# drowe67/pirip

Measured on AMD Instinct MI355X. Metric: IQ Msamples/s demodulated (2-FSK Fs=240k Rs=10k); BER vs CPU ref, higher is better.
Workload: dtype f32

## Files before the change

### pirip_amd/csrc/fsk_demod_wave.hip

```cpp
#include <hip/hip_runtime.h>

#include <cmath>
#include <cstdio>
#include <cstdlib>

#include "../../include/pirip_hip.h"
#include "demod_simd.hpp"
#include "fsk_device.hpp"

namespace pirip {

namespace {

constexpr int kWave = 64;

struct cf { float x, y; };

__device__ __forceinline__ float add_lane_up(float a, float b)
{
    float r;
    asm("v_add_f32_dpp %0, %1, %2 wave_shl:1 row_mask:0xf bank_mask:0xf bound_ctrl:0" : "=v"(r) : "v"(a), "v"(b));
    return r;
}

// ... 62 lines not shown
{
    const float hi = x * 0.00133514404296875f;
    return __builtin_fmaf(x, -0x1.e60f04p-20f, hi);
}
template <int FMT>
__device__ __forceinline__ v2f decode(const uint32_t *rw, int k)
{
    if (FMT == PIRIP_IN_CU8_FSKDEMOD || FMT == PIRIP_IN_CU8_CSDR) {
        const uint32_t v = rw[k >> 1];
        return cvt_u8_pair<FMT>(v2f{(k & 1) ? ubyte2(v) : ubyte0(v), (k & 1) ? ubyte3(v) : ubyte1(v)});
    } else if (FMT == PIRIP_IN_CS16) {
        const uint32_t v = rw[k];
        return v2f{cvt_s16((float)(short)(v & 0xffffu)), cvt_s16((float)((int)v >> 16))};
    } else {
        return v2f{__builtin_bit_cast(float, rw[2 * k]), __builtin_bit_cast(float, rw[2 * k + 1])};
    }
}
template <int FMT>
__device__ __forceinline__ v2f lds_sample(const unsigned char *p)
{
    if (FMT == PIRIP_IN_CU8_FSKDEMOD || FMT == PIRIP_IN_CU8_CSDR) {
        const uint32_t v = *(const uint16_t *)p;
        return cvt_u8_pair<FMT>(v2f{ubyte0(v), ubyte1(v)});
    } else if (FMT == PIRIP_IN_CS16) {
        const uint32_t v = *(const uint32_t *)p;
        return v2f{cvt_s16((float)(short)(v & 0xffffu)), cvt_s16((float)((int)v >> 16))};
    } else {
        const float2 v = *(const float2 *)p;
        return v2f{v.x, v.y};
    }
}

constexpr int cmax(int a, int b) { return a > b ? a : b; }

__device__ __forceinline__ float atan2_turns(float y, float x)
{
    const float ax = fabsf(x), ay = fabsf(y);
    const float mn = ax < ay ? ax : ay, mx = ax < ay ? ay : ax;
    const float t = mx > 0.f ? mn * __builtin_amdgcn_rcpf(mx) : 0.f;
    const float s1 = t * t, s2 = s1 * s1, s4 = s2 * s2;
    const float p01 = __builtin_fmaf(s1, -0.05304612219333649f, 0.15915483236312866f);
    const float p23 = __builtin_fmaf(s1, -0.02213626727461815f, 0.031745944172143936f);
    const float p45 = __builtin_fmaf(s1, -0.00889870710670948f, 0.015346021391451359f);
    const float p67 = __builtin_fmaf(s1, -0.0006453014793805778f, 0.0034795869141817093f);
    const float q0 = __builtin_fmaf(s2, p23, p01), q1 = __builtin_fmaf(s2, p67, p45);
    float r = __builtin_fmaf(s4, q1, q0) * t;
    r = ay > ax ? 0.25f - r : r;
    r = x < 0.f ? 0.5f - r : r;
    return __builtin_copysignf(r, y);
}

constexpr float kLlrMax = 24.0f;
__device__ __forceinline__ float ln_i0_tab(const float *tab, float x)
{
    const bool in = x < 32.0f;
    const float xs = (in ? x : 32.0f) * 8.0f;
    const int j = (int)xs;
    const float f = xs - (float)j;
    const float t0 = tab[j], t1 = tab[j + 1];
    return (t0 + (f * (t1 - t0))) + (in ? 0.0f : x - 32.0f);
}
__device__ __forceinline__ uint32_t spread16(uint32_t x)
{
    x = (x | (x << 8)) & 0x00FF00FFu; x = (x | (x << 4)) & 0x0F0F0F0Fu; x = (x | (x << 2)) & 0x33333333u; x = (x | (x << 1)) & 0x55555555u;
    return x;
}
// ... 33 lines not shown
    static constexpr int TAIL_DW = HIST * BPS / 4;
    static constexpr int TRAILER_DW = GUARD_B / 4;
    static_assert((HIST * BPS) % 4 == 0 && (GUARD_B - HIST * BPS) % 4 == 0, "tail copies move whole dwords");
    static_assert(GUARD_B + (2 * M + 1) * 4 <= M * HIST * 8, "the state block holds the raw tail and its trailer");
    static constexpr int CHS = (BPS == 2) ? TS : (TS % 8 == 0 ? 8 : TS % 4 == 0 ? 4 : 2);
    static constexpr int CH_DW = CHS * BPS / 4;
    static_assert(TS % 2 == 0 && TS % P == 0 && P >= 4, "bad Ts / P");
    static_assert(NLANES <= kWave, "one lane per symbol block");
    static_assert((TS * BPS) % 16 == 0 && (CHS * BPS) % 16 == 0 && TS % CHS == 0, "block and chunk strides keep 16-byte alignment");
    static_assert((N + Q) / (NDFT / 2) - 1 == NFFT && N / (NDFT / 2) - 1 == NFFT, "numffts must not depend on nin");
    static_assert(NDFT == 256 ? (NFFT >= 4) : NDFT == 512 ? (NFFT % 2 == 0) : (NDFT == 128 && NFFT <= 8),
                  "FFT batches (Ndft = 256: the last batch of 4 may be partial; Ndft = 128: one batch of up to eight)");
    static_assert((NFFT - 1) * (NDFT / 2) + NDFT <= N - Q, "FFT windows stay inside the shortest frame");
    static_assert(M * P <= 48, "window prefix sums are kept in registers");
};

template <class C, int M> constexpr int wave_lds_bytes() { return C::RAW_B + C::XP_B; }

}

template <int M, int TS, int P, int NSYM, int NDFT, int FMT, int WPB, int WPS, bool FFT_FMA = false, bool MASK = false, int BAND = 0>
__global__ __launch_bounds__(kWave * WPB, WPS) void fsk_demod_wave_kernel(DemodArgs a_kernarg, int nstreams)
{
    constexpr bool INPLACE = TS == 10;
    static_assert(offsetof(DemodArgs, d) == 0, "the argument block is the first kernel argument");
    auto ap = [&]() {
        if constexpr (INPLACE) return (const __attribute__((address_space(4))) DemodArgs *)__builtin_amdgcn_kernarg_segment_ptr();
        else return (const DemodArgs *)&a_kernarg;
    }();
#define PIRIP_ARGS_REREAD() do { if constexpr (INPLACE) asm volatile("" : "+s"(ap)); } while (0)
#define a (*ap)
#define d (ap->d)
    static_assert(BAND == 0 || ((BAND == 2 || BAND == 4) && NDFT == 256 && !MASK), "band-only estimator: Ndft = 256, peak method, 32 or 64 bins");
    auto cmul = [](v2f x, v2f t) { return FFT_FMA ? rot_step(x, t) : cmul_x(x, t); };
    using C = WaveCfg<M, TS, P, NSYM, NDFT, FMT>;
    constexpr int N = C::N, NMEM = C::NMEM, HIST = C::HIST, STEP = C::STEP, Q = C::Q, BPS = C::BPS;
    constexpr int GUARD_B = C::GUARD_B;

    __shared__ __attribute__((aligned(16))) unsigned char s_raw[WPB][C::RAW_B];
    __shared__ __attribute__((aligned(16))) unsigned char s_xp[WPB][C::XP_B];
    constexpr int TAB_F = NDFT == 256 ? 12 * 16 * 4 : NDFT == 512 ? 8 * 16 * 2 + 12 * 32 * 2 : 8 * 16 * 2;
    __shared__ __attribute__((aligned(16))) float s_tab[TAB_F];
    __shared__ __attribute__((aligned(16))) float2 s_tph[P];
    __shared__ __attribute__((aligned(16))) float2 s_tgain[NSYM + 2];
    __shared__ float s_misc[WPB][3];
    extern __shared__ __attribute__((aligned(16))) float s_lnI0[];

    const int lane0 = threadIdx.x & (kWave - 1);
    const int wv = __builtin_amdgcn_readfirstlane(threadIdx.x >> 6);
    const int sid = blockIdx.x * WPB + wv;

    if (NDFT == 256) {
        for (int i = threadIdx.x; i < 12 * 16; i += kWave * WPB)
            ((float4 *)s_tab)[i] = ((const float4 *)a.t.fast_tab)[(i & 15) * 12 + (i >> 4)];
    } else {
        for (int i = threadIdx.x; i < TAB_F / 4; i += kWave * WPB) ((float4 *)s_tab)[i] = ((const float4 *)(a.t.fast_tab + NDFT))[i];
    }
    if constexpr (P <= 10) if (a.io.soft.llr) {
        if (a.io.soft.llr_map == kLlrRician) { for (int i = threadIdx.x; i < 258; i += kWave * WPB) s_lnI0[i] = a.io.soft.lnI0[i]; }
        else if (threadIdx.x < 20) {
            const int sg = threadIdx.x >> 2, cc = threadIdx.x & 3;
            const float c2 = sg == 0 ? 0.226f : sg == 1 ? 0.1245f : sg == 2 ? 0.0288f : sg == 3 ? 0.002f : 0.0f;
            const float c1 = sg == 0 ? 0.0125f : sg == 1 ? 0.2177f : sg == 2 ? 0.6314f : sg == 3 ? 0.9048f : 0.9867f;
            const float c0 = sg == 0 ? -0.0012f : sg == 1 ? -0.108f : sg == 2 ? -0.5645f : sg == 3 ? -1.2997f : -2.2053f;
            s_lnI0[threadIdx.x] = cc == 0 ? c2 : cc == 1 ? c1 : cc == 2 ? c0 : 0.0f;
        }
// ... 550 lines not shown
            }
#pragma unroll
            for (int x = 1; x < M; x++)
#pragma unroll
                for (int y = x; y > 0; y--)
                    if (freqi[y] < freqi[y - 1]) { const int t = freqi[y]; freqi[y] = freqi[y - 1]; freqi[y - 1] = t; }
        }
        constexpr int LOG2N = NDFT == 128 ? 7 : NDFT == 256 ? 8 : 9;
        uint32_t dthv[M];
        int tix[M];
#pragma unroll
        for (int m = 0; m < M; m++) {
            if constexpr (MASK) { dthv[m] = a.t.mask_dtheta[bb * M + m]; tix[m] = bb * M + m; }
            else { dthv[m] = (uint32_t)freqi[m] << (32 - LOG2N); tix[m] = freqi[m] + NDFT / 2; }
        }

        auto phasor = [&](uint32_t th) {
            const float2 w = a.t.tw[th >> (32 - LOG2N)];
            float pc = w.x, ps = -w.y;
            if constexpr (MASK) {
                const float bl = (float)(th & ((1u << (32 - LOG2N)) - 1u)) * 1.4629180792671596e-9f;
                const float b2 = bl * bl;
                const float cb = 1.0f - b2 * (0.5f - b2 * (1.0f / 24.0f));
                const float sb = bl * (1.0f - b2 * ((1.0f / 6.0f) - b2 * (1.0f / 120.0f)));
                const float c2 = pc * cb - ps * sb, s2 = ps * cb + pc * sb;
                pc = c2; ps = s2;
            }
            return make_float2(pc, ps);
        };
        __builtin_amdgcn_sched_barrier(0);
        PIRIP_T_MARK(2);
        v2f fi[M][P];
        v2f tot[M];
        {
            PIRIP_PHASE_LANE(lane);
            const int lb = lane < C::NLANES ? lane : C::NLANES - 1;
            const int boff = GUARD_B + (TS * lb - nold) * BPS;
            const int al = (GUARD_B - nold * BPS) & 15;
            v2f ph[M], dph[M], acc[M];
            v2f sw_ph[M], sw_dph[M];
            const int n0 = TS * lb - nold + 1;
            const int nold_blk = nold - TS * lb;
            const bool oldl = nold_blk > 0;
#pragma unroll
            for (int m = 0; m < M; m++) {
                const float2 stn = a.t.osc_step[tix[m]], stp = a.t.osc_step[tixp[m]];
                const float dn = a.t.osc_drift[tix[m]].x, dp = a.t.osc_drift[tixp[m]].x;
                const uint32_t th = (uint32_t)n0 * (oldl ? dthp[m] : dthv[m]);
                const float g = 1.0f + (oldl ? dp * (float)(ninp + n0) : dn * (float)n0);
                const float2 pcs = phasor(th);
                ph[m] = v2f{pcs.x * g, pcs.y * g};
                dph[m] = oldl ? v2f{stp.x, stp.y} : v2f{stn.x, stn.y};
                const float2 p1 = phasor(dthv[m]);
                const float g1 = 1.0f + dn;
                sw_ph[m] = v2f{p1.x * g1, p1.y * g1};
                sw_dph[m] = v2f{stn.x, stn.y};
                acc[m] = v2f{0.f, 0.f};
            }
            const int zero_blk = ninp ? 0 : nold_blk;
#pragma unroll
            for (int c = 0; c < TS / C::CHS; c++) {
                uint32_t rw[C::CH_DW];
                if (C::DIRECT && lb >= 3) {
#pragma unroll
                    for (int i = 0; i < C::CH_DW / 4; i++) {
                        const auto v = __builtin_amdgcn_raw_buffer_load_b128(rsrc, (TS * lb - nold) * BPS + c * C::CHS * BPS + 16 * i, (int)goff_frame, 0);
                        const uint4 u = __builtin_bit_cast(uint4, v);
// ... 49 lines not shown
                    if ((kk & 3) == 3) __builtin_amdgcn_sched_barrier(0);
                }
            }
#pragma unroll
            for (int m = 0; m < M; m++) tot[m] = acc[m];
        }
        PIRIP_PHASE_LANE(lane);
        if constexpr (C::DIRECT) {
            asm volatile("s_waitcnt lgkmcnt(0)" ::: "memory");
            wave_lds_sync();
            const uint32_t toff = (uint32_t)__builtin_amdgcn_readfirstlane((int)(uint32_t)((pos + nin - HIST) * BPS));
#pragma unroll
            for (int i = 0; i < (C::TAIL_DW + kWave - 1) / kWave; i++)
                if (lane + i * kWave < C::TAIL_DW)
                    __builtin_amdgcn_raw_ptr_buffer_load_lds(rsrc, (lds_ptr)(raw + GUARD_B - HIST * BPS + i * 256), 4, lane * 4, toff + i * 256, 0, 0);
        } else {
            const uint32_t *tsrc = (const uint32_t *)(raw + GUARD_B + (nin - HIST) * BPS);
            uint32_t *tdst = (uint32_t *)(raw + GUARD_B - HIST * BPS);
            uint32_t tv[(C::TAIL_DW + kWave - 1) / kWave];
#pragma unroll
            for (int i = 0; i < (C::TAIL_DW + kWave - 1) / kWave; i++) tv[i] = tsrc[lane + i * kWave < C::TAIL_DW ? lane + i * kWave : 0];
#pragma unroll
            for (int i = 0; i < (C::TAIL_DW + kWave - 1) / kWave; i++) if (lane + i * kWave < C::TAIL_DW) tdst[lane + i * kWave] = tv[i];
        }
        asm volatile("s_waitcnt lgkmcnt(0)" ::: "memory");
        wave_lds_sync();
        PIRIP_T_MARK(3);
        dma_frame(pos + nin);
        ninp = nin;
#pragma unroll
        for (int m = 0; m < M; m++) { dthp[m] = dthv[m]; tixp[m] = tix[m]; }

        float tcr = 0.f, tci = 0.f;
        {
            v2f prpi{0.f, 0.f};
            v2f ft{0.f, 0.f};
#pragma unroll
            for (int q = 0; q < P; q++) {
#pragma unroll
                for (int m = 0; m < M; m++) {
                    const v2f own = fi[m][q];
                    v2f w0;
                    w0.x = add_lane_up(own.x, tot[m].x - own.x);
                    w0.y = add_lane_up(own.y, tot[m].y - own.y);
                    fi[m][q] = w0;
                    if (m == 0) asm("v_mul_f32 %0, %1, %1\n\tv_fma_f32 %0, %2, %2, %0" : "=&v"(ft.x) : "v"(w0.y), "v"(w0.x));
                    else { float t2; asm("v_mul_f32 %0, %2, %2\n\tv_fma_f32 %0, %3, %3, %0\n\tv_add_f32 %1, %1, %0" : "=&v"(t2), "+v"(ft.x) : "v"(w0.y), "v"(w0.x)); }
                }
                const v2f tp = *(const v2f *)&s_tph[q];
                asm("v_pk_fma_f32 %0, %1, %2, %0 op_sel_hi:[0,1,1]" : "+v"(prpi) : "v"(ft), "v"(tp));
                asm volatile("" : "+v"(prpi), "+v"(fi[0][q]), "+v"(fi[M - 1][q]));
            }
            const float pr = prpi.x, pi = prpi.y;
            if (lane <= NSYM) {
                const float2 tgain = s_tgain[lane];
                tcr = pr * tgain.x - pi * tgain.y;
                tci = pr * tgain.y + pi * tgain.x;
            }
            tcr = wave_sum(tcr); tci = wave_sum(tci);
        }

        PIRIP_T_MARK(4);
        PIRIP_ARGS_REREAD();
        const int frame_bytes = d.pack_bits ? (d.Nbits + 7) / 8 : d.Nbits;
        const size_t orow = (size_t)(frame + out0);
        uint8_t *bits_o = a.io.bits ? a.io.bits + (size_t)sid * a.io.bits_stride + orow * frame_bytes : nullptr;
        float *filt_o = a.io.filt ? a.io.filt + (size_t)sid * a.io.filt_stride + orow * M * NSYM : nullptr;
        float *stats_o = a.io.stats ? a.io.stats + (size_t)sid * a.io.stats_stride + orow * PIRIP_STATS_PER_FRAME : nullptr;
        float f_est[kMaxTones] = {0.f, 0.f, 0.f, 0.f};
#pragma unroll
        for (int m = 0; m < M; m++) {
            if constexpr (MASK) f_est[m] = (float)((bb - NDFT / 2) * d.Fs / NDFT) + (float)(m * d.tone_spacing);
            else f_est[m] = (float)freqi[m] * d.bin_hz;
        }

        const bool bad = isnan(tcr) || isnan(tci);
        int nin_next = nin;
        if (!bad) {
            const float norm_rx_timing = FMT == PIRIP_IN_CF32 ? atan2f(tci, tcr) * 0.15915494309189535f : atan2_turns(tci, tcr);
            const float rx_timing = norm_rx_timing * (float)P;
            const float d_norm = norm_rx_timing - sc_norm_rx_timing;
            sc_norm_rx_timing = norm_rx_timing;
            if (fabsf(d_norm) < 0.2f) {
                const float appm = (1e6f * d_norm) / (float)NSYM;
                sc_ppm = (0.9f * sc_ppm) + (0.1f * appm);
            }
            nin_next = N;
            if (!d.burst_mode) {
                if (norm_rx_timing > 0.25f) nin_next = N + Q;
                else if (norm_rx_timing < -0.25f) nin_next = N - Q;
            }

            const int low_sample = __builtin_amdgcn_readfirstlane((int)floorf(rx_timing));
            const float fract = rx_timing - (float)low_sample;
            const int high_sample = __builtin_amdgcn_readfirstlane((int)ceilf(rx_timing));
            v2f lo[M], hi[M];
            {
                const int ql = low_sample >= 0 ? low_sample : P + low_sample;
                const int qh = high_sample >= 0 ? high_sample : P + high_sample;
#define PIRIP_SEL_CASE(q) case q: if (q < P) { asm volatile(""); for (int m_ = 0; m_ < M; m_++) DST[m_] = fi[m_][q < P ? q : 0]; } break;
#define PIRIP_SELECT(idx) do { switch (idx) { \
    PIRIP_SEL_CASE(0) PIRIP_SEL_CASE(1) PIRIP_SEL_CASE(2) PIRIP_SEL_CASE(3) PIRIP_SEL_CASE(4) PIRIP_SEL_CASE(5) \
    PIRIP_SEL_CASE(6) PIRIP_SEL_CASE(7) PIRIP_SEL_CASE(8) PIRIP_SEL_CASE(9) PIRIP_SEL_CASE(10) PIRIP_SEL_CASE(11) \
    PIRIP_SEL_CASE(12) PIRIP_SEL_CASE(13) PIRIP_SEL_CASE(14) PIRIP_SEL_CASE(15) PIRIP_SEL_CASE(16) PIRIP_SEL_CASE(17) \
    PIRIP_SEL_CASE(18) PIRIP_SEL_CASE(19) PIRIP_SEL_CASE(20) PIRIP_SEL_CASE(21) PIRIP_SEL_CASE(22) PIRIP_SEL_CASE(23) \
    default: break; } } while (0)
                static_assert(P <= 24, "selection switch covers 24 window starts");
#pragma unroll
                for (int m = 0; m < M; m++) { lo[m] = fi[m][0]; hi[m] = fi[m][0]; }
#define DST lo
                PIRIP_SELECT(ql);
#undef DST
#define DST hi
                PIRIP_SELECT(qh);
#undef DST
#undef PIRIP_SELECT
#undef PIRIP_SEL_CASE
#pragma unroll
                for (int m = 0; m < M; m++) {
                    if (low_sample >= 0) { lo[m].x = lane_up(lo[m].x); lo[m].y = lane_up(lo[m].y); }
                    if (high_sample >= 0) { hi[m].x = lane_up(hi[m].x); hi[m].y = lane_up(hi[m].y); }
                }
            }
            float tmax[M];
            float sum = 0.f;
#pragma unroll
            for (int m = 0; m < M; m++) {
                v2f t;
                t.x = (1 - fract) * lo[m].x; t.y = (1 - fract) * lo[m].y;
                t.x = t.x + fract * hi[m].x; t.y = t.y + fract * hi[m].y;
// ... 132 lines not shown
        frame++;
        wave_lds_sync();
    }

    if constexpr (SOFT_OK) if (words_o && soft_cb > 0 && lane0 == 0) words_o[soft_w] = soft_carry;
    asm volatile("s_waitcnt vmcnt(0)" ::: "memory");
#ifdef PIRIP_WAVE_TIMING
    if (a.io.stats && lane0 == 0 && sid == nstreams / 2)
        for (int i = 0; i < 8; i++) a.io.stats[(size_t)sid * a.io.stats_stride + i] = (float)t_acc_[i];
#endif
#pragma unroll
    for (int b = 0; b < NB; b++) if (!BAND || lane0 < 16) a.s.Sf[(size_t)sid * NDFT + own_sfi(lane0, b)] = Sf[b];
    wave_lds_sync();
    for (int i = lane0; i < GUARD_B / 4; i += kWave) st32[i] = ((const uint32_t *)raw)[i];
    const int lane = lane0;
    if (lane == 0) {
#pragma unroll
        for (int m = 0; m < M; m++) { st32[C::TRAILER_DW + m] = dthp[m]; st32[C::TRAILER_DW + M + m] = (uint32_t)tixp[m]; }
        st32[C::TRAILER_DW + 2 * M] = (uint32_t)ninp;
        StreamScalars sc = a.s.scal[sid];
        sc.nin = nin; sc.norm_rx_timing = sc_norm_rx_timing; sc.ppm = sc_ppm; sc.SNRest = sc_SNRest;
        sc.snr_est = s_misc[wv][0]; sc.EbNodB = s_misc[wv][1]; sc.v_est = s_misc[wv][2];
        if (frame > frame_first) {
            const int fq[4] = {last_freqi0, last_freqi1, last_freqi2, last_freqi3};
            for (int m = 0; m < kMaxTones; m++) {
                if (MASK) sc.f_est[m] = m < M ? (float)((fq[0] - NDFT / 2) * d.Fs / NDFT) + (float)(m * d.tone_spacing) : 0.f;
                else sc.f_est[m] = m < M ? (float)fq[m] * d.bin_hz : 0.f;
            }
        }
        a.s.scal[sid] = sc;
        if (a.io.nframes) a.io.nframes[sid] = (int32_t)frame;
        if (a.io.consumed) a.io.consumed[sid] = pos;
    }
#undef a
#undef d
#undef PIRIP_ARGS_REREAD
}

namespace {
__global__ void sqrt_selftest_kernel(unsigned long long *bad, unsigned lo, unsigned hi)
{
    unsigned long long c = 0;
    const unsigned stride = gridDim.x * blockDim.x;
    for (unsigned long long b = (unsigned long long)lo + blockIdx.x * blockDim.x + threadIdx.x; b <= hi; b += stride) {
        const float x = __builtin_bit_cast(float, (unsigned)b);
        const float want = (float)sqrt((double)x);
        if (__builtin_bit_cast(unsigned, sqrt_rn_normal<true>(x)) != __builtin_bit_cast(unsigned, want)) c++;
        if (x != 0.0f && __builtin_bit_cast(unsigned, sqrt_rn_normal<true, true>(x)) != __builtin_bit_cast(unsigned, want)) c++;
        if (__builtin_bit_cast(unsigned, sqrt_rn_normal<false>(x)) != __builtin_bit_cast(unsigned, want)) c += 1ull << 32;
    }
    if (c) atomicAdd(bad, c);
}
}

hipError_t selftest_sqrt(unsigned long long *mismatches)
{
    unsigned long long *d = nullptr;
    hipError_t e = hipMalloc(&d, sizeof(*d));
    if (e != hipSuccess) return e;
    e = hipMemset(d, 0, sizeof(*d));
    if (e == hipSuccess) {
        hipLaunchKernelGGL(sqrt_selftest_kernel, dim3(4096), dim3(256), 0, 0, d, 0u, 0u);
        hipLaunchKernelGGL(sqrt_selftest_kernel, dim3(4096), dim3(256), 0, 0, d, 0x0f800000u, 0x7f7fffffu);
        e = hipMemcpy(mismatches, d, sizeof(*d), hipMemcpyDeviceToHost);
        if (e == hipSuccess) e = hipGetLastError();
    }
// ... 137 lines not shown
```

### pirip_amd/csrc/fsk_plan.cpp

```cpp
#include "fsk_plan.hpp"

#include <cassert>
#include <cmath>
#include <cstdlib>
#include <cstring>
#include <string>

#include "../../include/pirip_hip.h"

namespace pirip {

namespace {
struct cf { float re, im; };
inline cf cmul(cf a, cf b) { return {a.re * b.re - a.im * b.im, a.re * b.im + a.im * b.re}; }
}

int FskPlan::init(int Fs, int Rs, int M, int P, int Nsym, int est_min, int est_max,
                  int freq_est_type, int tone_spacing, int in_format, const pirip_fsk_recalled *recalled)
{
    pirip_fsk_recalled rc;
    recalled_defaults(&rc);
    const pirip_fsk_recalled dflt = rc;
    if (recalled) rc = *recalled;
    if (!(rc.tc > 0.0f && rc.tc <= 1.0f) || !(rc.est_space_rs >= 0.0f) || !(rc.nin_threshold > 0.0f && rc.nin_threshold < 0.5f) || rc.nin_step_div < 2 ||
// ... 136 lines not shown

    {
        const int per = d.freq_est_type ? M : 1;
        osc_drift.assign(2 * (size_t)Ndft * per, 0.f);
        osc_step.assign(2 * (size_t)Ndft * per, 0.f);
        for (int b = 0; b < Ndft; b++) {
            for (int m = 0; m < per; m++) {
                float f_est; double ideal_turns;
                if (d.freq_est_type) {
                    const float foff = (float)((b - Ndft / 2) * Fs / Ndft);
                    f_est = foff + (float)(m * tone_spacing);
                    ideal_turns = 0.0;
                } else {
                    f_est = (float)(b - Ndft / 2) * d.bin_hz;
                    ideal_turns = (double)(b - Ndft / 2) / Ndft;
                }
                const float w = 2 * M_PI * ((f_est) / (float)(Fs));
                const float c = cosf(w), s = sinf(w);
                if (d.freq_est_type) {
                    double turns = std::atan2((double)s, (double)c) / (2.0 * M_PI);
                    turns -= std::floor(turns);
                    const uint32_t step = (uint32_t)((uint64_t)std::llround(turns * 4294967296.0) & 0xffffffffull);
                    mask_dtheta[(size_t)b * M + m] = step;
                    ideal_turns = (double)step / 4294967296.0;
                }
                const double a = std::sqrt((double)c * c + (double)s * s) - 1.0;
                double dd = std::atan2((double)s, (double)c) - 2.0 * M_PI * ideal_turns;
                dd -= 2.0 * M_PI * std::round(dd / (2.0 * M_PI));
                const size_t ix = 2 * ((size_t)b * per + m);
                osc_drift[ix] = (float)a; osc_drift[ix + 1] = (float)dd;
                osc_step[ix] = c; osc_step[ix + 1] = s;
            }
        }
        timing_rec.resize(2 * (size_t)d.nint);
        const float wt = 2 * M_PI * ((float)(Rs) / (float)(P * Rs));
        cf dph{cosf(wt), sinf(wt)}, ph{1.0f, 0.0f};
        for (int i = 0; i < d.nint; i++) {
            timing_rec[2 * i] = ph.re; timing_rec[2 * i + 1] = ph.im;
            ph = cmul(ph, dph);
        }
    }
    fast_tab.clear();
    for (auto &v : tw_s2) v = 0.f;
    if (Ndft == 256) {
        fast_tab.assign(16 * 48, 0.f);
        for (int e = 0; e < 16; e++) {
            float *row = &fast_tab[(size_t)e * 48];
            const int a = e >> 2, b = e & 3, base = a + 4 * b;
            for (int t = 0; t < 16; t++) row[t] = hann[base + 16 * t];
            for (int r = 1; r <= 3; r++) {
                row[16 + 2 * (r - 1)] = twiddle[2 * (4 * e * r)];
                row[16 + 2 * (r - 1) + 1] = twiddle[2 * (4 * e * r) + 1];
            }
            for (int bp = 0; bp < 4; bp++)
                for (int r = 1; r <= 3; r++) {
                    const int k = (e + 16 * bp) * r;
                    row[22 + 2 * (3 * bp + (r - 1))] = twiddle[2 * k];
                    row[22 + 2 * (3 * bp + (r - 1)) + 1] = twiddle[2 * k + 1];
                }
        }
        for (int k = 1; k <= 3; k++)
            for (int r = 1; r <= 3; r++) {
                tw_s2[2 * (3 * (k - 1) + (r - 1))] = twiddle[2 * (16 * k * r)];
                tw_s2[2 * (3 * (k - 1) + (r - 1)) + 1] = twiddle[2 * (16 * k * r) + 1];
            }
    }
// ... 21 lines not shown
                    p3[2 * ((3 * jj + (j - 1)) * 32 + L)] = twiddle[2 * k];
                    p3[2 * ((3 * jj + (j - 1)) * 32 + L) + 1] = twiddle[2 * k + 1];
                }
        for (int j = 1; j <= 3; j++) { tw_s2[2 * (j - 1)] = twiddle[2 * (64 * j)]; tw_s2[2 * (j - 1) + 1] = twiddle[2 * (64 * j) + 1]; }
    }
    if (Ndft == 128) {
        fast_tab.assign(128 + 8 * 16 * 2, 0.f);
        for (int i = 0; i < 128; i++) fast_tab[i] = hann[i];
        float *p2 = &fast_tab[128];
        for (int r = 0; r < 8; r++) {
            for (int j = 1; j <= 3; j++) {
                p2[2 * (r * 16 + (j - 1))] = twiddle[2 * (4 * r * j)];
                p2[2 * (r * 16 + (j - 1)) + 1] = twiddle[2 * (4 * r * j) + 1];
            }
            for (int j1 = 0; j1 < 4; j1++)
                for (int j = 1; j <= 3; j++) {
                    const int k = (r + 8 * j1) * j;
                    p2[2 * (r * 16 + 3 + 3 * j1 + (j - 1))] = twiddle[2 * k];
                    p2[2 * (r * 16 + 3 + 3 * j1 + (j - 1)) + 1] = twiddle[2 * k + 1];
                }
        }
        for (int j = 1; j <= 3; j++) { tw_s2[2 * (j - 1)] = twiddle[2 * (16 * j)]; tw_s2[2 * (j - 1) + 1] = twiddle[2 * (16 * j) + 1]; }
    }
    if (Ndft == 4096) {
        fast_tab.assign(16 * 256 * 2, 0.f);
        for (int i = 0; i < 15; i++)
            for (int t = 0; t < 256; t++) {
                const int k4 = i < 3 ? 0 : (i - 3) / 3, r = i < 3 ? i + 1 : (i - 3) % 3 + 1;
                const int k = i < 3 ? 4 * t * r : (t + 256 * k4) * r;
                fast_tab[2 * (i * 256 + t)] = twiddle[2 * k]; fast_tab[2 * (i * 256 + t) + 1] = twiddle[2 * k + 1];
            }
    }
    return PIRIP_OK;
}

bool fsk_est_range(int Fs, int Ndft, int est_min, int est_max, int *st_out, int *en_out)
{
    if (est_min == 0 && est_max == 0) { est_min = 0; est_max = Fs; }
    else if (est_min < -Fs / 2 || est_max > Fs / 2 || est_max <= est_min) return false;
    int st = (est_min * Ndft) / Fs + Ndft / 2; if (st < 0) st = 0;
    int en = (est_max * Ndft) / Fs + Ndft / 2; if (en > Ndft) en = Ndft;
    *st_out = st; *en_out = en;
    return true;
}

void FskMod::init(int Fs_, int Rs_, int M_, int f1, int spacing)
{
    Fs = Fs_; Rs = Rs_; M = M_; Ts = Fs_ / Rs_; f1_tx = f1; tone_spacing = spacing;
    ph_re = cosf(0); ph_im = sinf(0);
}

void FskMod::mod(const uint8_t *bits, int nbits, float *out, bool complex_out)
{
    cf dosc[kMaxTones];
    for (int m = 0; m < M; m++) {
        const float w = 2 * M_PI * ((float)(f1_tx + (tone_spacing * m)) / (float)(Fs));
        dosc[m] = cf{cosf(w), sinf(w)};
    }
    const int bps = (M == 2) ? 1 : 2;
    const int nsym = nbits / bps;
    cf ph{ph_re, ph_im};
    int bit_i = 0;
    for (int i = 0; i < nsym; i++) {
        int sym = 0;
        for (int b = 0; b < bps; b++) sym = (sym << 1) | (bits[bit_i++] == 1 ? 1 : 0);
        const cf dph = dosc[sym];
// ... 116 lines not shown
```

### pirip_amd/csrc/fsk_plan.hpp

```cpp
#pragma once
#include <cstdint>
#include <vector>

#include "../../include/pirip_hip.h"

namespace pirip {

constexpr int kMaxTones = 4;
constexpr int kMaxStages = 16;

struct FftStage { int radix; int m; int fstride; };

struct FskDims {
    int Fs, Rs, M, P, Nsym;
    int Ts, N, Nmem, Ndft, Nbits, nint;
    int est_st, est_en, f_zero;
    int freq_est_type;
    int tone_spacing;
    int mask_len;
    int n_teeth;
    int in_format;
    int hist_len;
    int grp;
    int nstages;
    int pack_bits;
    int burst_mode;
    int fft_fma;
    int est_band;
    float tc, one_minus_tc;
    float bin_hz;
    int nin_step;
    float nin_thresh;
    float s16_scale;
    int u8_table;
    int sf_power;
    int recalled_fast_ok;
    int block_stagger;
};

struct FskPlan {
    FskDims d{};
    FftStage stages[kMaxStages]{};
    std::vector<float> hann;
    std::vector<float> twiddle;
    std::vector<uint16_t> leaf_perm;
    std::vector<uint16_t> leaf_iperm;
    std::vector<float> u8_lut;
    std::vector<float> timing_ph;
    std::vector<int16_t> teeth;
    std::vector<uint32_t> mask_dtheta;
    std::vector<float> osc_drift;
    std::vector<float> osc_step;
    std::vector<float> timing_rec;
    std::vector<float> fast_tab;
    float tw_s2[18];
    int init(int Fs, int Rs, int M, int P, int Nsym, int est_min, int est_max,
             int freq_est_type, int tone_spacing, int in_format, const pirip_fsk_recalled *recalled = nullptr);
};

struct FskMod {
    int Fs, Rs, M, Ts, f1_tx, tone_spacing;
    float ph_re = 1.0f, ph_im = 0.0f;
    void init(int Fs_, int Rs_, int M_, int f1, int spacing);
    void mod(const uint8_t *bits, int nbits, float *out, bool complex_out);
};

void test_frame_bits(uint8_t *frame, int framesize);

struct PutBits {
    int framesize; float valid_thresh;
    std::vector<uint8_t> tx, rx;
    long bitcnt = 0, biterr = 0; int packetcnt = 0;
    void init(int framesize_, float valid_thresh_);
    bool push(uint8_t bit, int *errs_out);
    float ber() const { return bitcnt ? (float)biterr / (float)bitcnt : 0.5f; }
};

int csdr_filter_len(float transition_bw);
void csdr_lowpass_hamming(float *taps, int length, float cutoff_rate);
void csdr_lowpass(float *taps, int length, float cutoff_rate, int window);
bool fsk_est_range(int Fs, int Ndft, int est_min, int est_max, int *st, int *en);
void recalled_defaults(pirip_fsk_recalled *r);
bool recalled_from_env(pirip_fsk_recalled *r);

}
// ... 1 lines not shown
```

### pirip_amd/csrc/pirip_capi.hip

```cpp
#include <hip/hip_runtime.h>

#include <cstdio>
#include <cstdlib>
#include <cstring>
#include <new>
#include <vector>

#include "../../include/pirip_hip.h"
#include "fsk_device.hpp"
#include "fsk_plan.hpp"
#include "demod_handle.hpp"

using namespace pirip;

#define HIPCHK(expr)                                              \
    do {                                                          \
        hipError_t e_ = (expr);                                   \
        if (e_ != hipSuccess) {                                   \
            h->last_hip = (int)e_;                                \
            return PIRIP_ERR_HIP;                                 \
        }                                                         \
    } while (0)


// ... 168 lines not shown
    h->nstreams = nstreams;
    {
        const char *k = getenv("PIRIP_KERNEL");
        const bool want_general = getenv("PIRIP_FORCE_GENERAL") || (k && !strcmp(k, "general"));
        if (const char *f = getenv("PIRIP_FFT_FMA")) {
            h->plan.d.fft_fma = atoi(f) ? 1 : 0;
            if (h->plan.d.fft_fma && !demod_wave_applicable(h->plan.d)) h->plan.d.fft_fma = 0;
        }
        h->kernel = want_general || !h->plan.d.recalled_fast_ok ? 0 :
                    demod_wave_applicable(h->plan.d) ? PIRIP_KERNEL_WAVE : demod_block_applicable(h->plan.d) ? PIRIP_KERNEL_BLOCK : 0;
        if (const char *sg = getenv("PIRIP_BLOCK_STAGGER")) h->plan.d.block_stagger = atoi(sg) > 0 ? atoi(sg) : 0;
        if (const char *b = getenv("PIRIP_EST_BAND")) {
            if (atoi(b)) h->plan.d.est_band = est_band_for(h);
        }
        if (k && !strcmp(k, "exact")) {
            h->plan.d.grp = 1;
            if (!demod_exact_applicable(h->plan.d)) { delete h; return PIRIP_ERR_UNSUPPORTED; }
            h->kernel = PIRIP_KERNEL_EXACT;
        }
    }

    const FskPlan &pl = h->plan;
    const FskDims &d = pl.d;
    const size_t ns = (size_t)nstreams;
    bool ok = true;
    ok &= upload(&h->d_hann, pl.hann.data(), sizeof(float) * d.Ndft) == hipSuccess;
    ok &= upload(&h->d_tw, pl.twiddle.data(), sizeof(float) * 2 * d.Ndft) == hipSuccess;
    ok &= upload(&h->d_perm, pl.leaf_iperm.data(), sizeof(uint16_t) * d.Ndft) == hipSuccess;
    ok &= upload(&h->d_lut, pl.u8_lut.data(), sizeof(float) * 256) == hipSuccess;
    ok &= upload(&h->d_tph, pl.timing_ph.data(), sizeof(float) * 2 * d.P) == hipSuccess;
    ok &= upload(&h->d_teeth, pl.teeth.data(), sizeof(int16_t) * pl.teeth.size()) == hipSuccess;
    ok &= upload(&h->d_mask_dtheta, pl.mask_dtheta.data(), sizeof(uint32_t) * pl.mask_dtheta.size()) == hipSuccess;
    ok &= upload(&h->d_osc_drift, pl.osc_drift.data(), sizeof(float) * pl.osc_drift.size()) == hipSuccess;
    ok &= upload(&h->d_osc_step, pl.osc_step.data(), sizeof(float) * pl.osc_step.size()) == hipSuccess;
    ok &= upload(&h->d_timing_rec, pl.timing_rec.data(), sizeof(float) * pl.timing_rec.size()) == hipSuccess;
    ok &= upload(&h->d_fast_tab, pl.fast_tab.data(), sizeof(float) * pl.fast_tab.size()) == hipSuccess;
    ok &= hipMalloc((void **)&h->d_Sf, sizeof(float) * ns * d.Ndft) == hipSuccess;
    ok &= hipMalloc((void **)&h->d_theta, sizeof(uint32_t) * ns * kMaxTones) == hipSuccess;
    ok &= hipMalloc((void **)&h->d_hist, sizeof(float2) * ns * d.M * d.hist_len) == hipSuccess;
    ok &= hipMalloc((void **)&h->d_scal, sizeof(StreamScalars) * ns) == hipSuccess;
    ok &= hipMalloc((void **)&h->d_first, sizeof(int32_t) * ns) == hipSuccess;
    ok &= hipMalloc((void **)&h->d_phic, sizeof(float2) * ns * kMaxTones) == hipSuccess;
    if (!ok) { free_all(h); delete h; return PIRIP_ERR_NOMEM; }
    if (const char *e = getenv("PIRIP_EXACT0")) h->exact0 = atoi(e) ? 1 : 0;
    rc = reset_state(h, nullptr);
    if (rc != PIRIP_OK) { free_all(h); delete h; return rc; }
    *out = h;
    return PIRIP_OK;
}

int pirip_hip_destroy(pirip_hip_demod *h)
{
    if (!h) return PIRIP_ERR_BAD_ARG;
    (void)bind(h);
    (void)hipDeviceSynchronize();
    pirip::capture_release(h);
    free_all(h);
    delete h;
    return PIRIP_OK;
}

int pirip_hip_get_kernel(const pirip_hip_demod *h) { return h ? h->kernel : PIRIP_ERR_BAD_ARG; }

int pirip_hip_get_kernel_name(const pirip_hip_demod *h, char *buf, size_t n)
{
    if (!h || !buf || !n) return PIRIP_ERR_BAD_ARG;
    buf[0] = 0;
// ... 345 lines not shown
```

Baseline: 355,100.

## Compute tone-mixer integrate-and-dump correlations with f16 MFMA using hi/lo split tables

For the common config (2 tones, Ts=P=24, Nsym=50, Ndft=256, cu8 input), the per-sample oscillator mix and integrate step is recast as a matrix multiply. The host precomputes a per-bin table of rotating phasor coefficients, split into fp16 hi and lo parts and appended to the osc_step buffer. The kernel converts u8 samples to fp16 and runs 32x32x16 f16 MFMAs to produce all timing-phase filter outputs at once. Timing estimation and sample picking are rewritten to read the MFMA accumulator layout, with permlane swaps and a separate amplitude-drift gain correction. The path runs only when the tone indices match the previous frame, so it adds a second code path with tighter precision margins.

```diff
diff --git a/pirip_amd/csrc/fsk_demod_wave.hip b/pirip_amd/csrc/fsk_demod_wave.hip
--- a/pirip_amd/csrc/fsk_demod_wave.hip
+++ b/pirip_amd/csrc/fsk_demod_wave.hip
@@ -118,6 +118,23 @@
 }
 
 constexpr int cmax(int a, int b) { return a > b ? a : b; }
+
+typedef _Float16 h2v __attribute__((ext_vector_type(2)));
+typedef _Float16 h8v __attribute__((ext_vector_type(8)));
+typedef float f16v __attribute__((ext_vector_type(16)));
+constexpr int kCorrPad = 7, kCorrRow = 40;
+__device__ __forceinline__ void u8x4_to_h4(uint32_t w, uint32_t &o0, uint32_t &o1)
+{
+    const h2v sc{(_Float16)0.0078125f, (_Float16)0.0078125f}, of{(_Float16)-8.9921875f, (_Float16)-8.9921875f};
+    const uint32_t p0 = __builtin_amdgcn_perm(0x64646464u, w, 0x04010400u), p1 = __builtin_amdgcn_perm(0x64646464u, w, 0x04030402u);
+    o0 = __builtin_bit_cast(uint32_t, __builtin_elementwise_fma(__builtin_bit_cast(h2v, p0), sc, of));
+    o1 = __builtin_bit_cast(uint32_t, __builtin_elementwise_fma(__builtin_bit_cast(h2v, p1), sc, of));
+}
+__device__ __forceinline__ void swap_halves(float &a, float &b)
+{
+    const auto r = __builtin_amdgcn_permlane32_swap(__builtin_bit_cast(unsigned, a), __builtin_bit_cast(unsigned, b), false, false);
+    a = __builtin_bit_cast(float, r[0]); b = __builtin_bit_cast(float, r[1]);
+}
 
 __device__ __forceinline__ float atan2_turns(float y, float x)
 {
@@ -217,6 +234,7 @@
 #define a (*ap)
 #define d (ap->d)
     static_assert(BAND == 0 || ((BAND == 2 || BAND == 4) && NDFT == 256 && !MASK), "band-only estimator: Ndft = 256, peak method, 32 or 64 bins");
+    constexpr bool CORR_MX = M == 2 && TS == 24 && P == 24 && NSYM == 50 && NDFT == 256 && FMT == PIRIP_IN_CU8_FSKDEMOD && !FFT_FMA && !MASK && BAND == 0;
     auto cmul = [](v2f x, v2f t) { return FFT_FMA ? rot_step(x, t) : cmul_x(x, t); };
     using C = WaveCfg<M, TS, P, NSYM, NDFT, FMT>;
     constexpr int N = C::N, NMEM = C::NMEM, HIST = C::HIST, STEP = C::STEP, Q = C::Q, BPS = C::BPS;
@@ -833,7 +851,51 @@
         PIRIP_T_MARK(2);
         v2f fi[M][P];
         v2f tot[M];
-        {
+        bool corr_mx = false;
+        if constexpr (CORR_MX) corr_mx = ninp != 0 && tix[0] == tixp[0] && tix[M - 1] == tixp[M - 1];
+        const int ninp_frame = ninp;
+        if constexpr (CORR_MX) if (corr_mx) {
+            PIRIP_PHASE_LANE(lane);
+            const int r = lane & 31, hh = lane >> 5;
+            const uint32_t *ctab = (const uint32_t *)(a.t.osc_step + NDFT) + (((r & 2) ? tix[M - 1] : tix[0]) * 4 + (r & 1) * 2) * kCorrRow
+                                   + (kCorrPad + 4 * hh - (r >> 2));
+            auto afrag = [&](int D, int hl) { uint4 v; __builtin_memcpy(&v, ctab + hl * kCorrRow + 8 * D, 16); return __builtin_bit_cast(h8v, v); };
+            h8v Ah[4];
+#pragma unroll
+            for (int D = 0; D < 4; D++) Ah[D] = afrag(D, 0);
+            f16v acc[2][3];
+#pragma unroll
+            for (int i = 0; i < 6; i++)
+#pragma unroll
+                for (int j = 0; j < 16; j++) acc[i / 3][i % 3][j] = 0.f;
+            const int b0 = r, b1 = 32 + r <= NSYM ? 32 + r : NSYM;
+            const unsigned char *p0 = raw + GUARD_B + (TS * b0 - nold) * BPS + 8 * hh, *p1 = raw + GUARD_B + (TS * b1 - nold) * BPS + 8 * hh;
+#pragma unroll
+            for (int ks = 0; ks < 6; ks++) {
+                h8v Al[3];
+#pragma unroll
+                for (int t = 0; t < 3; t++) if (ks - t >= 0 && ks - t <= 3) Al[t] = afrag(ks - t, 1);
+#pragma unroll
+                for (int ct = 0; ct < 2; ct++) {
+                    const uint32_t *bp = (const uint32_t *)((ct ? p1 : p0) + 16 * ks);
+                    uint4 xb;
+                    u8x4_to_h4(bp[0], xb.x, xb.y);
+                    u8x4_to_h4(bp[1], xb.z, xb.w);
+                    const h8v X = __builtin_bit_cast(h8v, xb);
+#pragma unroll
+                    for (int t = 0; t < 3; t++) {
+                        if (ks - t < 0 || ks - t > 3) continue;
+                        acc[ct][t] = __builtin_amdgcn_mfma_f32_32x32x16_f16(Ah[ks - t], X, acc[ct][t], 0, 0, 0);
+                        acc[ct][t] = __builtin_amdgcn_mfma_f32_32x32x16_f16(Al[t], X, acc[ct][t], 0, 0, 0);
+                    }
+                }
+                __builtin_amdgcn_sched_barrier(0);
+            }
+#pragma unroll
+            for (int i = 0; i < 48; i++) fi[i / P][i % P] = v2f{acc[i / 24][(i / 8) % 3][(2 * i) % 16], acc[i / 24][(i / 8) % 3][(2 * i) % 16 + 1]};
+            tot[0] = tot[M - 1] = v2f{0.f, 0.f};
+        }
+        if (!(CORR_MX && corr_mx)) {
             PIRIP_PHASE_LANE(lane);
             const int lb = lane < C::NLANES ? lane : C::NLANES - 1;
             const int boff = GUARD_B + (TS * lb - nold) * BPS;
@@ -949,7 +1011,48 @@
         for (int m = 0; m < M; m++) { dthp[m] = dthv[m]; tixp[m] = tix[m]; }
 
         float tcr = 0.f, tci = 0.f;
-        {
+#define PIRIP_MXW(ct, t, g, m) fi[(((ct) * 3 + (t)) * 8 + 2 * (g) + (m)) / P][(((ct) * 3 + (t)) * 8 + 2 * (g) + (m)) % P]
+        auto win_gain = [&](float slope, int n0, int oldw) { return 1.0f + slope * ((float)n0 + (float)(ninp_frame * oldw) * (1.0f / (float)TS)); };
+        if constexpr (CORR_MX) if (corr_mx) {
+            const int r = lane & 31, hh = lane >> 5;
+            const int nold_f = NMEM - nin;
+            v2f pp[2][M];
+#pragma unroll
+            for (int ct = 0; ct < 2; ct++) {
+                pp[ct][0] = pp[ct][M - 1] = v2f{0.f, 0.f};
+#pragma unroll
+                for (int i = 0; i < 12; i++) {
+                    const v2f tp = *(const v2f *)&s_tph[2 * i + hh];
+#pragma unroll
+                    for (int m = 0; m < M; m++) {
+                        const v2f w0 = PIRIP_MXW(ct, i >> 2, i & 3, m);
+                        v2f ft;
+                        asm("v_mul_f32 %0, %1, %1\n\tv_fma_f32 %0, %2, %2, %0" : "=&v"(ft.x) : "v"(w0.y), "v"(w0.x));
+                        ft.y = 0.f;
+                        asm("v_pk_fma_f32 %0, %1, %2, %0 op_sel_hi:[0,1,1]" : "+v"(pp[ct][m]) : "v"(ft), "v"(tp));
+                    }
+                }
+            }
+#pragma unroll
+            for (int ct = 0; ct < 2; ct++) {
+                const int blk = 32 * ct + r;
+                if (blk <= NSYM) {
+                    const int n0 = TS * blk - nold_f + 1 + TS / 2;
+                    int oldw = nold_f - TS * blk - TS / 2; oldw = oldw < 0 ? 0 : oldw > TS ? TS : oldw;
+                    float pr = 0.f, pi = 0.f;
+#pragma unroll
+                    for (int m = 0; m < M; m++) {
+                        const float g = win_gain(a.t.osc_drift[tixp[m]].x, n0, oldw), g2 = g * g;
+                        pr += g2 * pp[ct][m].x; pi += g2 * pp[ct][m].y;
+                    }
+                    const float2 tgain = s_tgain[blk];
+                    tcr += pr * tgain.x - pi * tgain.y;
+                    tci += pr * tgain.y + pi * tgain.x;
+                }
+            }
+            tcr = wave_sum(tcr); tci = wave_sum(tci);
+        }
+        if (!(CORR_MX && corr_mx)) {
             v2f prpi{0.f, 0.f};
             v2f ft{0.f, 0.f};
 #pragma unroll
@@ -1012,7 +1115,51 @@
             const float fract = rx_timing - (float)low_sample;
             const int high_sample = __builtin_amdgcn_readfirstlane((int)ceilf(rx_timing));
             v2f lo[M], hi[M];
-            {
+            if constexpr (CORR_MX) if (corr_mx) {
+                const int ql = low_sample >= 0 ? low_sample : P + low_sample;
+                const int qh = high_sample >= 0 ? high_sample : P + high_sample;
+                const int nold_f = NMEM - nin;
+                auto pick = [&](int q, v2f *dst) {
+                    v2f e[2][M];
+#pragma unroll
+                    for (int ct = 0; ct < 2; ct++) e[ct][0] = e[ct][M - 1] = v2f{0.f, 0.f};
+#define PIRIP_MX_CASE(i) case i: asm volatile(""); for (int ct_ = 0; ct_ < 2; ct_++) for (int m_ = 0; m_ < M; m_++) e[ct_][m_] = PIRIP_MXW(ct_, (i) >> 2, (i) & 3, m_); break;
+                    switch (q >> 1) {
+                        PIRIP_MX_CASE(0) PIRIP_MX_CASE(1) PIRIP_MX_CASE(2) PIRIP_MX_CASE(3) PIRIP_MX_CASE(4) PIRIP_MX_CASE(5)
+                        PIRIP_MX_CASE(6) PIRIP_MX_CASE(7) PIRIP_MX_CASE(8) PIRIP_MX_CASE(9) PIRIP_MX_CASE(10) PIRIP_MX_CASE(11)
+                        default: break;
+                    }
+#undef PIRIP_MX_CASE
+                    const bool odd = q & 1;
+                    const int n0 = TS * lane - nold_f + 1 + q;
+                    int oldw = nold_f - TS * lane - q; oldw = oldw < 0 ? 0 : oldw > TS ? TS : oldw;
+#pragma unroll
+                    for (int m = 0; m < M; m++) {
+                        float ex0 = e[0][m].x, ex1 = e[1][m].x, ey0 = e[0][m].y, ey1 = e[1][m].y;
+                        swap_halves(ex0, ex1); swap_halves(ey0, ey1);
+                        const float g = win_gain(a.t.osc_drift[tixp[m]].x, n0, oldw);
+                        dst[m] = v2f{(odd ? ex1 : ex0) * g, (odd ? ey1 : ey0) * g};
+                    }
+                };
+                pick(ql, lo);
+                if (qh != ql) {
+                    pick(qh, hi);
+#pragma unroll
+                    for (int m = 0; m < M; m++) {
+                        const float2 stp = a.t.osc_step[tixp[m]];
+                        hi[m] = v2f{hi[m].x * stp.x + hi[m].y * stp.y, hi[m].y * stp.x - hi[m].x * stp.y};
+                    }
+                } else {
+#pragma unroll
+                    for (int m = 0; m < M; m++) hi[m] = lo[m];
+                }
+#pragma unroll
+                for (int m = 0; m < M; m++) {
+                    if (low_sample >= 0) { lo[m].x = lane_up(lo[m].x); lo[m].y = lane_up(lo[m].y); }
+                    if (high_sample >= 0) { hi[m].x = lane_up(hi[m].x); hi[m].y = lane_up(hi[m].y); }
+                }
+            }
+            if (!(CORR_MX && corr_mx)) {
                 const int ql = low_sample >= 0 ? low_sample : P + low_sample;
                 const int qh = high_sample >= 0 ? high_sample : P + high_sample;
 #define PIRIP_SEL_CASE(q) case q: if (q < P) { asm volatile(""); for (int m_ = 0; m_ < M; m_++) DST[m_] = fi[m_][q < P ? q : 0]; } break;
@@ -1211,6 +1358,7 @@
         if (a.io.nframes) a.io.nframes[sid] = (int32_t)frame;
         if (a.io.consumed) a.io.consumed[sid] = pos;
     }
+#undef PIRIP_MXW
 #undef a
 #undef d
 #undef PIRIP_ARGS_REREAD
diff --git a/pirip_amd/csrc/fsk_plan.cpp b/pirip_amd/csrc/fsk_plan.cpp
--- a/pirip_amd/csrc/fsk_plan.cpp
+++ b/pirip_amd/csrc/fsk_plan.cpp
@@ -192,6 +192,8 @@
                 osc_step[ix] = c; osc_step[ix + 1] = s;
             }
         }
+        corr_tab.clear();
+        if (!d.freq_est_type && M == 2 && Ndft == 256 && d.Ts == kCorrTaps && P == kCorrTaps && !build_corr_tab()) return PIRIP_ERR_UNSUPPORTED;
         timing_rec.resize(2 * (size_t)d.nint);
         const float wt = 2 * M_PI * ((float)(Rs) / (float)(P * Rs));
         cf dph{cosf(wt), sinf(wt)}, ph{1.0f, 0.0f};
@@ -279,6 +281,54 @@
             }
     }
     return PIRIP_OK;
+}
+
+static uint16_t to_half(double x, double *back)
+{
+    const double ax = std::fabs(x);
+    int e = 0;
+    if (ax != 0.0) (void)std::frexp(ax, &e);
+    const int q = (e - 1 < -14 ? -14 : e - 1) - 10;
+    const double n = std::nearbyint(std::ldexp(ax, -q));
+    const double r = std::ldexp(n, q);
+    *back = x < 0 ? -r : r;
+    uint32_t bits;
+    if (n < 1024.0) bits = (uint32_t)n;
+    else { int e2; const double f2 = std::frexp(r, &e2); bits = ((uint32_t)(e2 - 1 + 15) << 10) | ((uint32_t)std::ldexp(f2, 11) & 0x3ffu); }
+    return (uint16_t)(bits | (x < 0 ? 0x8000u : 0u));
+}
+
+bool FskPlan::build_corr_tab()
+{
+    const int Ndft = d.Ndft;
+    corr_tab.assign((size_t)Ndft * 4 * kCorrRow, 0u);
+    for (int b = 0; b < Ndft; b++) {
+        const float cf_ = osc_step[2 * (size_t)b], sf_ = osc_step[2 * (size_t)b + 1];
+        const double c1 = cf_, s1 = sf_;
+        double pc = 1.0, ps = 0.0;
+        float fc = 1.0f, fs = 0.0f;
+        for (int t = 0; t < kCorrTaps; t++) {
+            if (std::fabs(pc - (double)fc) > 4e-6 || std::fabs(ps - (double)fs) > 4e-6) return false;
+            const double coef[2][2] = {{pc, ps}, {-ps, pc}};
+            for (int c = 0; c < 2; c++) {
+                uint16_t hi[2], lo[2];
+                for (int k = 0; k < 2; k++) {
+                    double bh, bl;
+                    hi[k] = to_half(coef[c][k], &bh);
+                    lo[k] = to_half(coef[c][k] - bh, &bl);
+                    if (std::fabs(bh + bl - coef[c][k]) > kCorrSplitTol) return false;
+                }
+                uint32_t *row = &corr_tab[((size_t)b * 2 + c) * 2 * kCorrRow];
+                row[t + kCorrPad] = (uint32_t)hi[0] | ((uint32_t)hi[1] << 16);
+                row[kCorrRow + t + kCorrPad] = (uint32_t)lo[0] | ((uint32_t)lo[1] << 16);
+            }
+            const double nc = pc * c1 - ps * s1, ns = pc * s1 + ps * c1;
+            pc = nc; ps = ns;
+            const float gc = std::fmaf(-fs, sf_, fc * cf_), gs = std::fmaf(fs, cf_, fc * sf_);
+            fc = gc; fs = gs;
+        }
+    }
+    return true;
 }
 
 bool fsk_est_range(int Fs, int Ndft, int est_min, int est_max, int *st_out, int *en_out)
diff --git a/pirip_amd/csrc/fsk_plan.hpp b/pirip_amd/csrc/fsk_plan.hpp
--- a/pirip_amd/csrc/fsk_plan.hpp
+++ b/pirip_amd/csrc/fsk_plan.hpp
@@ -51,6 +51,10 @@
     std::vector<uint32_t> mask_dtheta;
     std::vector<float> osc_drift;
     std::vector<float> osc_step;
+    static constexpr int kCorrPad = 7, kCorrRow = 40, kCorrTaps = 24;
+    static constexpr double kCorrSplitTol = 0x1p-23;
+    std::vector<uint32_t> corr_tab;
+    bool build_corr_tab();
     std::vector<float> timing_rec;
     std::vector<float> fast_tab;
     float tw_s2[18];
diff --git a/pirip_amd/csrc/pirip_capi.hip b/pirip_amd/csrc/pirip_capi.hip
--- a/pirip_amd/csrc/pirip_capi.hip
+++ b/pirip_amd/csrc/pirip_capi.hip
@@ -224,7 +224,12 @@
     ok &= upload(&h->d_teeth, pl.teeth.data(), sizeof(int16_t) * pl.teeth.size()) == hipSuccess;
     ok &= upload(&h->d_mask_dtheta, pl.mask_dtheta.data(), sizeof(uint32_t) * pl.mask_dtheta.size()) == hipSuccess;
     ok &= upload(&h->d_osc_drift, pl.osc_drift.data(), sizeof(float) * pl.osc_drift.size()) == hipSuccess;
-    ok &= upload(&h->d_osc_step, pl.osc_step.data(), sizeof(float) * pl.osc_step.size()) == hipSuccess;
+    {
+        std::vector<uint32_t> buf(pl.osc_step.size() + pl.corr_tab.size());
+        std::memcpy(buf.data(), pl.osc_step.data(), sizeof(float) * pl.osc_step.size());
+        if (!pl.corr_tab.empty()) std::memcpy(buf.data() + pl.osc_step.size(), pl.corr_tab.data(), sizeof(uint32_t) * pl.corr_tab.size());
+        ok &= upload(&h->d_osc_step, buf.data(), sizeof(uint32_t) * buf.size()) == hipSuccess;
+    }
     ok &= upload(&h->d_timing_rec, pl.timing_rec.data(), sizeof(float) * pl.timing_rec.size()) == hipSuccess;
     ok &= upload(&h->d_fast_tab, pl.fast_tab.data(), sizeof(float) * pl.fast_tab.size()) == hipSuccess;
     ok &= hipMalloc((void **)&h->d_Sf, sizeof(float) * ns * d.Ndft) == hipSuccess;
```

Result: slower. 302,000, median of 2 (-14.9%).
